# VIS4ROB-lab/ccm_slam

Hardware: AMD Instinct MI355X
Metric: global-BA LM iterations/s (4-agent merged map) (higher is better)
Workload: dtype f64; 1 GPU; gba_c4: global BA (MapFusionGBA numerics), 2000 KFs / 150000 landmarks / 954782 observations, Huber sqrt(5.99), landmark-sharded x1

## Files before the change

### ccm_slam_amd/csrc/ba_build.hip

```cpp
#include "common.h"
#include "ba_types.h"
#include "ba_math.h"
#include <algorithm>
#include <chrono>
#include <cstring>
#include <rocprim/rocprim.hpp>

int ccm_ba_build_pairs(ccm_ctx* ctx, const int* d_pt_off, const int* d_cslot, int Lp, int Cp, int lb, int le, int eb,
                       uint32_t** d_U_out, int* nOff_out, int** d_inst_off, int** d_inst_a, int** d_inst_c, int64_t* n_inst,
                       std::vector<std::pair<void*, size_t>>& keep);
int ccm_ba_pers_grid_fits(ccm_ctx* ctx, int grid);
int ccm_ba_state_from_raw(ccm_ba* ba);

namespace {

constexpr int kB = 256;

inline double now_ms() { return std::chrono::duration<double, std::milli>(std::chrono::steady_clock::now().time_since_epoch()).count(); }

struct BuildSizes {
  int Cp, Lp, Eact, bad, max_cam_edges, n_fix_edges, worst_units, n_units, pers_bad, n_ucol, n_cij, ncb, pad[4];
};

#define BB_RC(x) do { int rc_ = (x); if (rc_) return rc_; } while (0)
#define BB_HIP(x) do { hipError_t e_ = (x); if (e_ != hipSuccess) return ccm_set_error(ctx, CCM_E_HIP, std::string(#x) + ": " + hipGetErrorString(e_)); } while (0)

struct Tmp {
  ccm_ctx* ctx;
  std::vector<std::pair<void*, size_t>> blocks;
  template <typename T> int get(size_t n, T** out) {
    void* p = nullptr; size_t actual = 0;
    if (int rc = ccm_pool_get(ctx, std::max<size_t>(n, 1) * sizeof(T), &p, &actual)) return rc;
    blocks.push_back({p, actual});
    *out = (T*)p;
    return CCM_OK;
  }
  ~Tmp() { hipStreamSynchronize(ctx->stream); for (auto& b : blocks) ccm_pool_put(ctx, b.first, b.second); }
};

template <typename T>
int keep_get(ccm_ba* ba, size_t n, T** out, bool zero = false) {
  ccm_ctx* ctx = ba->ctx;
  void* p = nullptr; size_t actual = 0;
  const size_t bytes = std::max<size_t>(n, 1) * sizeof(T);
  if (int rc = ccm_pool_get(ctx, bytes, &p, &actual)) return rc;
  ba->allocs.push_back({p, actual});
  if (zero) ba->zero_list.push_back({p, bytes});
  *out = (T*)p;
  return CCM_OK;
}

constexpr int kZeroMax = 96;
constexpr unsigned kZeroChunk16 = 4096;
struct ZeroTab { void* p[kZeroMax]; unsigned n16[kZeroMax]; unsigned first_chunk[kZeroMax + 1]; int n; };
__global__ __launch_bounds__(256) void bb_zero_many(ZeroTab tab) {
  int k = 0;
  while (k + 1 < tab.n && blockIdx.x >= tab.first_chunk[k + 1]) k++;
  const unsigned c = blockIdx.x - tab.first_chunk[k];
  uint4* q = reinterpret_cast<uint4*>(tab.p[k]);
  const unsigned end = min(tab.n16[k], (c + 1) * kZeroChunk16);
  for (unsigned i = c * kZeroChunk16 + threadIdx.x; i < end; i += 256) q[i] = make_uint4(0u, 0u, 0u, 0u);
}
int flush_zero_list(ccm_ba* ba) {
  ccm_ctx* ctx = ba->ctx;
  size_t k = 0;
  while (k < ba->zero_list.size()) {
    ZeroTab tab;
    tab.n = 0;
    unsigned chunks = 0;
    for (; k < ba->zero_list.size() && tab.n < kZeroMax; k++) {
      const size_t n16 = (ba->zero_list[k].second + 15) / 16;
      if (n16 > 0xffffffffull / 2) { BB_HIP(hipMemsetAsync(ba->zero_list[k].first, 0, ba->zero_list[k].second, ctx->stream)); continue; }
      tab.p[tab.n] = ba->zero_list[k].first; tab.n16[tab.n] = (unsigned)n16; tab.first_chunk[tab.n] = chunks;
      chunks += (unsigned)((n16 + kZeroChunk16 - 1) / kZeroChunk16);
      tab.n++;
    }
    tab.first_chunk[tab.n] = chunks;
    if (chunks) hipLaunchKernelGGL(bb_zero_many, dim3(chunks), dim3(256), 0, ctx->stream, tab);
    BB_HIP(hipGetLastError());
  }
  ba->zero_list.clear();
  return CCM_OK;
}

int scan_excl(ccm_ctx* ctx, Tmp& tmp, const int* in, int* out, size_t n) {
  size_t bytes = 0;
  BB_HIP(rocprim::exclusive_scan(nullptr, bytes, in, out, 0, n, rocprim::plus<int>(), ctx->stream));
  char* scratch = nullptr;
  BB_RC(tmp.get(bytes, &scratch));
  BB_HIP(rocprim::exclusive_scan(scratch, bytes, in, out, 0, n, rocprim::plus<int>(), ctx->stream));
  return CCM_OK;
}

template <typename K>
int sort_pairs(ccm_ctx* ctx, Tmp& tmp, K* keys, int* vals, size_t n, unsigned bits, K** keys_sorted, int** vals_sorted) {
  *keys_sorted = keys; *vals_sorted = vals;
  if (n == 0) return CCM_OK;
  K* k2 = nullptr; int* v2 = nullptr;
  BB_RC(tmp.get(n, &k2)); BB_RC(tmp.get(n, &v2));
  rocprim::double_buffer<K> kb(keys, k2);
  rocprim::double_buffer<int> vb(vals, v2);
  size_t bytes = 0;
  BB_HIP(rocprim::radix_sort_pairs(nullptr, bytes, kb, vb, (unsigned)n, 0u, bits, ctx->stream));
  char* scratch = nullptr;
  BB_RC(tmp.get(bytes, &scratch));
  BB_HIP(rocprim::radix_sort_pairs(scratch, bytes, kb, vb, (unsigned)n, 0u, bits, ctx->stream));
  *keys_sorted = kb.current(); *vals_sorted = vb.current();
  return CCM_OK;
}

inline unsigned bits_for(uint64_t n_values) {
  unsigned b = 1;
  while (b < 63 && ((uint64_t)1 << b) < n_values) b++;
  return b;
}

__global__ void bb_mark(int n_edge, const int* ecam, const int* ept, const uint8_t* lvl, int n_cam, int n_pt, int* cam_has, int* pt_has, BuildSizes* sz) {
  const int e = blockIdx.x * blockDim.x + threadIdx.x;
  if (e >= n_edge) return;
  const int c = ecam[e], p = ept[e];
  if (c < 0 || c >= n_cam || p < 0 || p >= n_pt) { sz->bad = 1; return; }
  if (lvl && lvl[e] != 0) return;
  cam_has[c] = 1; pt_has[p] = 1;
}

__global__ void bb_flags(int n, const int* has, const uint8_t* fixed, int* flag) {
  const int i = blockIdx.x * blockDim.x + threadIdx.x;
  if (i > n) return;
  flag[i] = (i < n && has[i] && !(fixed && fixed[i])) ? 1 : 0;
}

__global__ void bb_slots(int n, const int* flag, const int* pre, int* slot, int* inv, int* total) {
  const int i = blockIdx.x * blockDim.x + threadIdx.x;
  if (i > n) return;
  if (i == n) { *total = pre[n]; return; }
  const int f = flag[i];
  slot[i] = f ? pre[i] : -1;
  if (f) inv[pre[i]] = i;
}

__global__ void bb_keys(int n_edge, const int* ecam, const int* ept, const uint8_t* lvl, int n_cam, int n_pt, const int* cam_slot, const int* pt_slot, unsigned cb,
                        unsigned pb, unsigned long long* keys, int* vals) {
  const int e = blockIdx.x * blockDim.x + threadIdx.x;
  if (e >= n_edge) return;
  const bool in_range = ecam[e] >= 0 && ecam[e] < n_cam && ept[e] >= 0 && ept[e] < n_pt;
  const bool act = in_range && !(lvl && lvl[e] != 0);
  unsigned long long k = (((unsigned long long)1 << (pb + cb)) - 1ull);
  if (act) k = ((unsigned long long)(unsigned)pt_slot[ept[e]] << cb) | (unsigned long long)(unsigned)(cam_slot[ecam[e]] + 1);
  keys[e] = k;
  vals[e] = e;
}

__global__ void bb_ptoff(int n_edge, const unsigned long long* keys, unsigned cb, unsigned pb, int* pt_off, int* cslot_g, BuildSizes* sz) {
  const int k = blockIdx.x * blockDim.x + threadIdx.x;
  if (k >= n_edge) return;
  const unsigned long long sent = ((unsigned long long)1 << pb) - 1ull;
  const unsigned long long cur = keys[k] >> cb;
  if (cur == sent) return;
  cslot_g[k] = (int)(keys[k] & (((unsigned long long)1 << cb) - 1ull)) - 1;
  const unsigned long long nxt = (k + 1 < n_edge) ? (keys[k + 1] >> cb) : sent;
  if (nxt != cur) pt_off[cur + 1] = k + 1;
  if (nxt == sent) sz->Eact = k + 1;
}

__global__ void bb_weights(int Lp, const int* pt_off, const int* cslot_g, long long* w) {
  const int l = blockIdx.x * blockDim.x + threadIdx.x;
  if (l >= Lp) return;
  int kf = 0;
  for (int k = pt_off[l]; k < pt_off[l + 1]; k++) kf += cslot_g[k] >= 0;
  w[l] = (long long)kf * (kf + 1) / 2 + (pt_off[l + 1] - pt_off[l]);
}

__global__ void bb_ptoff_local(int n, const int* g_pt_off, int eb, int* pt_off) {
  const int l = blockIdx.x * blockDim.x + threadIdx.x;
  if (l < n) pt_off[l] = g_pt_off[l] - eb;
}

__global__ void bb_gather(int Eloc, int eb, int lb, const unsigned long long* keys, const int* vals, unsigned cb, const int* ecam, const double* obs_raw,
                          const double* info_raw, int* ed_cam, int* ed_cslot, int* ed_pt, double* obs, double* info, int* loc_orig, unsigned* ckey, int* cval) {
  const int k = blockIdx.x * blockDim.x + threadIdx.x;
  if (k >= Eloc) return;
  const unsigned long long key = keys[eb + k];
  const int e = vals[eb + k];
  const int cs = (int)(key & (((unsigned long long)1 << cb) - 1ull)) - 1;
  ed_cam[k] = ecam[e]; ed_cslot[k] = cs; ed_pt[k] = (int)(key >> cb) - lb;
  obs[2 * (size_t)k] = obs_raw[2 * (size_t)e]; obs[2 * (size_t)k + 1] = obs_raw[2 * (size_t)e + 1];
  info[k] = info_raw[e];
  loc_orig[k] = e;
  ckey[k] = (unsigned)(cs + 1); cval[k] = k;
}

__global__ void bb_lower_bound(const unsigned* a, int n, int nq, int* off) {
  const int s = blockIdx.x * blockDim.x + threadIdx.x;
  if (s >= nq) return;
  int lo = 0, hi = n;
  while (lo < hi) { const int mid = (lo + hi) >> 1; if (a[mid] < (unsigned)s) lo = mid + 1; else hi = mid; }
  off[s] = lo;
}

__global__ void bb_cam_lists(int Eloc, const int* off_all , const int* cval, const int* ed_pt, int* cam_edge, int* cam_pt) {
  const int q = blockIdx.x * blockDim.x + threadIdx.x;
  const int nfix = off_all[1];
  if (q >= Eloc - nfix) return;
  const int k = cval[nfix + q];
  cam_edge[q] = k; cam_pt[q] = ed_pt[k];
}
__global__ void bb_cam_oi_bounded(int Eloc, const int* __restrict__ off_all, const int* __restrict__ cam_edge, const double* __restrict__ obs, const double* __restrict__ info,
                                  double* __restrict__ cam_oi) {
  const int s = blockIdx.x * blockDim.x + threadIdx.x;
  if (s >= Eloc - off_all[1]) return;
  const int e = cam_edge[s];
  typedef double v2d __attribute__((ext_vector_type(2)));
  v2d a, b; a[0] = obs[2 * (size_t)e]; a[1] = obs[2 * (size_t)e + 1]; b[0] = info[e]; b[1] = 0.0;
  reinterpret_cast<v2d*>(cam_oi)[2 * (size_t)s] = a; reinterpret_cast<v2d*>(cam_oi)[2 * (size_t)s + 1] = b;
}
__global__ void bb_cam_off(int Cp, const int* off_all, int* cam_off, BuildSizes* sz) {
  const int i = blockIdx.x * blockDim.x + threadIdx.x;
  if (i > Cp) return;
  cam_off[i] = off_all[i + 1] - off_all[1];
  if (i < Cp) atomicMax(&sz->max_cam_edges, off_all[i + 2] - off_all[i + 1]);
  if (i == 0) sz->n_fix_edges = off_all[1];
}

__global__ void bb_block_ij(int nOff, const uint32_t* U, int Cp, int* bi, int* bj, unsigned* jkey, int* jval) {
  const int b = blockIdx.x * blockDim.x + threadIdx.x;
  if (b >= nOff) return;
  const uint32_t u = U[b];
  const int i = (int)(u / (uint32_t)Cp), j = (int)(u % (uint32_t)Cp);
  bi[Cp + b] = i; bj[Cp + b] = j;
  jkey[b] = (unsigned)j; jval[b] = b;
}
__global__ void bb_diag_ij(int Cp, int* bi, int* bj) {
  const int i = blockIdx.x * blockDim.x + threadIdx.x;
  if (i < Cp) { bi[i] = i; bj[i] = i; }
}
__global__ void bb_rowblk_off(int Cp, const uint32_t* U, int nOff, int* rowblk_off) {
  const int i = blockIdx.x * blockDim.x + threadIdx.x;
  if (i > Cp) return;
  const unsigned long long key = (unsigned long long)i * (unsigned long long)Cp;
  int lo = 0, hi = nOff;
  while (lo < hi) { const int mid = (lo + hi) >> 1; if ((unsigned long long)U[mid] < key) lo = mid + 1; else hi = mid; }
  rowblk_off[i] = lo;
}
__global__ void bb_row_off(int Cp, const int* rowblk_off, const int* low_off, int* row_off) {
  const int i = blockIdx.x * blockDim.x + threadIdx.x;
  if (i <= Cp) row_off[i] = i + rowblk_off[i] + low_off[i];
}
__global__ void bb_row_fill(int Cp, int nOff, const int* bi, const int* bj, const unsigned* jkey_sorted, const int* jval_sorted, const int* rowblk_off,
                            const int* low_off, const int* row_off, int* row_col, uint32_t* row_blk) {
  const int t = blockIdx.x * blockDim.x + threadIdx.x;
  if (t < nOff) {
    {
      const int j = (int)jkey_sorted[t], b = jval_sorted[t];
      const int pos = row_off[j] + (t - low_off[j]);
      row_col[pos] = bi[Cp + b]; row_blk[pos] = (uint32_t)(Cp + b) | kTransposeBit;
    }
    {
      const int i = bi[Cp + t];
      const int pos = row_off[i] + (low_off[i + 1] - low_off[i]) + 1 + (t - rowblk_off[i]);
      row_col[pos] = bj[Cp + t]; row_blk[pos] = (uint32_t)(Cp + t);
    }
  }
  if (t < Cp) {
    const int pos = row_off[t] + (low_off[t + 1] - low_off[t]);
    row_col[pos] = t; row_blk[pos] = (uint32_t)t;
  }
}

__device__ __forceinline__ void pers_unit_rows(int u, int Cp, int& r0, int& r1) {
  r0 = min(Cp, (u >> 1) * kClu + (u & 1) * (kClu / 2));
  r1 = min(min(Cp, r0 + kClu / 2), ((u >> 1) + 1) * kClu);
}
template <int FILL>
__global__ __launch_bounds__(kB) void bb_pers_units(int Cp, int n_words, const int* row_off, const int* row_col, int* ucnt, const int* uoff, int* ucol, int* loc,
                                                  BuildSizes* sz) {
  extern __shared__ unsigned bm[];
  unsigned* wpre = bm + n_words;
  __shared__ int s_tot;
  const int u = blockIdx.x, t = threadIdx.x;
  int r0, r1;
  pers_unit_rows(u, Cp, r0, r1);
  for (int w = t; w < n_words; w += kB) bm[w] = 0u;
  __syncthreads();
  const int e0 = row_off[r0], e1 = row_off[r1];
  for (int s = e0 + t; s < e1; s += kB) { const int c = row_col[s]; atomicOr(&bm[c >> 5], 1u << (c & 31)); }
  __syncthreads();
  if (t == 0) {
    int acc = 0;
    for (int w = 0; w < n_words; w++) { wpre[w] = (unsigned)acc; acc += __popc(bm[w]); }
    s_tot = acc;
  }
  __syncthreads();
  if (!FILL) {
    if (t == 0) { ucnt[u] = s_tot; if (s_tot > kPersColCap || e1 - e0 > kPersIdxCap) sz->pers_bad = 1; }
    return;
  }
  const int base = uoff[u];
  for (int w = t; w < n_words; w += kB) {
    unsigned m = bm[w];
    int pos = base + (int)wpre[w];
    while (m) { const int b = __ffs(m) - 1; ucol[pos++] = 32 * w + b; m &= m - 1; }
  }
  for (int s = e0 + t; s < e1; s += kB) { const int c = row_col[s]; loc[s] = (int)wpre[c >> 5] + __popc(bm[c >> 5] & ((1u << (c & 31)) - 1u)); }
}

template <int FILL>
__global__ __launch_bounds__(kB) void bb_cluster_entries(int Cp, const int* row_off, const int* row_col, const uint32_t* row_blk, int* ccnt, const int* coff, int* cij,
                                                       uint32_t* cblk) {
  __shared__ int s_scan[kB];
  __shared__ int s_run;
  const int c = blockIdx.x, t = threadIdx.x;
  const int r0 = c * kClu, r1 = min(Cp, r0 + kClu);
  const int e0 = row_off[r0], e1 = row_off[r1];
  if (t == 0) s_run = 0;
  __syncthreads();
  for (int sb = e0; sb < e1; sb += kB) {
    const int s = sb + t;
    int col = -1;
    if (s < e1) col = row_col[s];
    const int in = (s < e1 && col >= r0 && col < r1) ? 1 : 0;
    s_scan[t] = in;
    __syncthreads();
    for (int off = 1; off < kB; off <<= 1) {
      const int v = (t >= off) ? s_scan[t - off] : 0;
      __syncthreads();
      s_scan[t] += v;
      __syncthreads();
    }
    const int run = s_run;
    if (FILL && in) {
      int lo = r0, hi = r1;
      while (hi - lo > 1) { const int mid = (lo + hi) >> 1; if (row_off[mid] <= s) lo = mid; else hi = mid; }
      const int pos = coff[c] + run + s_scan[t] - 1;
      cij[pos] = ((lo - r0) << 4) | (col - r0);
      cblk[pos] = row_blk[s];
    }
    __syncthreads();
    if (t == kB - 1) s_run = run + s_scan[kB - 1];
    __syncthreads();
  }
  if (!FILL && t == 0) ccnt[c] = s_run;
}

__global__ void bb_unit_counts(int nOff, int chunk, const int* inst_off, int* nub) {
  const int t = blockIdx.x * blockDim.x + threadIdx.x;
  if (t <= nOff) nub[t] = (t < nOff) ? max(1, (inst_off[t + 1] - inst_off[t] + chunk - 1) / chunk) : 0;
}
__global__ void bb_unit_offsets(int nOff, int Cp, const int* blk_pref, const int* rowblk_off, int* row_unit_off, int* blk_unit0, BuildSizes* sz) {
  const int t = blockIdx.x * blockDim.x + threadIdx.x;
  if (t <= Cp) row_unit_off[t] = blk_pref[rowblk_off[t]];
  if (t < Cp) atomicMax(&sz->worst_units, blk_pref[rowblk_off[t + 1]] - blk_pref[rowblk_off[t]]);
  if (t == 0) sz->n_units = blk_pref[nOff];
  if (t <= nOff) blk_unit0[t] = blk_pref[t];
}
__global__ __launch_bounds__(kB) void bb_unit_fill(int Cp, int chunk, const int* rowblk_off, const int* inst_off, const int* row_unit_off, const int* blk_unit0, int4* tab) {
  extern __shared__ int su[];
  const int i = blockIdx.x, t = threadIdx.x;
  const int base = row_unit_off[i], n = row_unit_off[i + 1] - base;
  int* blk = su; int* s0a = su + n; int* s1a = su + 2 * n;
  for (int b = rowblk_off[i] + t; b < rowblk_off[i + 1]; b += kB) {
    int c = blk_unit0[b] - base, s0 = inst_off[b];
    const int end = inst_off[b + 1];
    do { const int s1 = min(end, s0 + chunk); blk[c] = b; s0a[c] = s0; s1a[c] = s1; c++; s0 = s1; } while (s0 < end);
  }
  __syncthreads();
  for (int c = t; c < n; c += kB) {
    const int len = s1a[c] - s0a[c];
    int rank = 0;
    for (int o = 0; o < n; o++) { const int lo = s1a[o] - s0a[o]; rank += (lo > len || (lo == len && o < c)) ? 1 : 0; }
    tab[base + rank] = make_int4(blk[c], s0a[c], s1a[c], c);
  }
}

__global__ void bb_edge_rank(const int* cam_off, const int* cam_edge, int* rank) {
  const int i = blockIdx.x;
  for (int s = cam_off[i] + threadIdx.x; s < cam_off[i + 1]; s += blockDim.x) rank[cam_edge[s]] = s - cam_off[i];
}
__global__ void bb_inst_rank(const int* inst_a, const int* rank, int n, int* inst_al) {
  const int s = blockIdx.x * blockDim.x + threadIdx.x;
  if (s < n) inst_al[s] = rank[inst_a[s]];
}
__global__ void bb_edge_cpos(const int* cam_off, const int* cam_edge, int* cpos) {
  const int i = blockIdx.x;
  for (int s = cam_off[i] + threadIdx.x; s < cam_off[i + 1]; s += blockDim.x) cpos[cam_edge[s]] = s;
}
__global__ void bb_inst_cpos(const int* inst_c, const int* cpos, int n, int* inst_cp) {
  const int s = blockIdx.x * blockDim.x + threadIdx.x;
  if (s < n) inst_cp[s] = cpos[inst_c[s]];
}

__global__ void bb_coarse_keys(int Cp, int nOff, const int* bi, const int* bj, int na, int agg, unsigned* keys, int* vals) {
  const int k = blockIdx.x * blockDim.x + threadIdx.x;
  if (k >= Cp + nOff) return;
  const int a = bi[k] / agg, a2 = bj[k] / agg;
  keys[k] = (unsigned)a * (unsigned)na + (unsigned)a2;
  vals[k] = (k < Cp) ? 2 * k : 2 * k + (a == a2 ? 1 : 0);
}
__global__ void bb_coarse_ab(const unsigned* uniq, const int* n_runs, int na, int* cb_ab, BuildSizes* sz) {
  const int r = blockIdx.x * blockDim.x + threadIdx.x;
  if (r == 0) sz->ncb = *n_runs;
  if (r >= *n_runs) return;
  cb_ab[2 * r] = (int)(uniq[r] / (unsigned)na); cb_ab[2 * r + 1] = (int)(uniq[r] % (unsigned)na);
}
__global__ void bb_counts_tail(unsigned* counts, const int* n_runs) { counts[*n_runs] = 0u; }

__global__ void bb_state_init(int n_cam, int Lloc, int lb, const double* raw_cam, const double* raw_pt, const int* slot_pt, double* cam0, double* cam1, double* pt0,
                              double* pt1) {
  const int t = blockIdx.x * blockDim.x + threadIdx.x;
  if (t < n_cam) {
// ... 422 lines not shown
```

### ccm_slam_amd/csrc/ba_structure.hip

```cpp
#include "common.h"
#include <cstring>
#include <rocprim/rocprim.hpp>
#include <vector>

namespace {

constexpr int kTPB = 256;

template <int EMIT>
__global__ void pairs_kernel(const int* pt_off, const int* cslot, int l0, int n_l, int Cp, int* cnt, const int* poff, uint32_t* keys,
                             unsigned long long* vals) {
  const int i = blockIdx.x * blockDim.x + threadIdx.x;
  if (i >= n_l) return;
  const int l = l0 + i;
  const int k0 = pt_off[l], k1 = pt_off[l + 1];
  int n = 0;
  int w = EMIT ? poff[i] : 0;
  for (int a = k0; a < k1; a++) {
    const int ia = cslot[a];
    if (ia < 0) continue;
    for (int c = a + 1; c < k1; c++) {
      const int ic = cslot[c];
      if (ic == ia) continue;
      if (EMIT) { keys[w] = (uint32_t)ia * (uint32_t)Cp + (uint32_t)ic; if (vals) vals[w] = ((unsigned long long)(uint32_t)a << 32) | (uint32_t)c; w++; }
      n++;
    }
  }
  if (!EMIT) cnt[i] = n;
}

__global__ void split_kernel(const unsigned long long* vals, int n, int eb, int* inst_a, int* inst_c) {
  const int i = blockIdx.x * blockDim.x + threadIdx.x;
  if (i >= n) return;
  inst_a[i] = (int)(vals[i] >> 32) - eb;
  inst_c[i] = (int)(uint32_t)vals[i] - eb;
}

__global__ void ranges_kernel(const uint32_t* U, int nOff, const uint32_t* own_keys, int n_own, int* inst_off) {
  const int b = blockIdx.x * blockDim.x + threadIdx.x;
  if (b > nOff) return;
  if (b == nOff) { inst_off[b] = n_own; return; }
  const uint32_t key = U[b];
  int lo = 0, hi = n_own;
  while (lo < hi) { const int mid = (lo + hi) >> 1; if (own_keys[mid] < key) lo = mid + 1; else hi = mid; }
  inst_off[b] = lo;
}

struct Tmp {
  ccm_ctx* ctx;
  std::vector<std::pair<void*, size_t>> blocks;
  template <typename T> int get(size_t n, T** out) {
    void* p = nullptr; size_t actual = 0;
    if (int rc = ccm_pool_get(ctx, std::max<size_t>(n, 1) * sizeof(T), &p, &actual)) return rc;
    blocks.push_back({p, actual});
    *out = (T*)p;
    return CCM_OK;
  }
  ~Tmp() { hipStreamSynchronize(ctx->stream); for (auto& b : blocks) ccm_pool_put(ctx, b.first, b.second); }
};

#define ST_RC(x) do { int rc_ = (x); if (rc_) return rc_; } while (0)
#define ST_HIP(x) do { hipError_t e_ = (x); if (e_ != hipSuccess) return ccm_set_error(ctx, CCM_E_HIP, std::string(#x) + ": " + hipGetErrorString(e_)); } while (0)

int emit_pairs(ccm_ctx* ctx, Tmp& tmp, const int* d_pt_off, const int* d_cslot, int l0, int l1, int Cp, bool with_vals, uint32_t** keys,
               unsigned long long** vals, int* n_out) {
  const int n_l = l1 - l0;
  *keys = nullptr; if (vals) *vals = nullptr; *n_out = 0;
  if (n_l <= 0) return CCM_OK;
  int *cnt = nullptr, *poff = nullptr;
  ST_RC(tmp.get((size_t)n_l + 1, &cnt)); ST_RC(tmp.get((size_t)n_l + 1, &poff));
  ST_HIP(hipMemsetAsync(cnt + n_l, 0, sizeof(int), ctx->stream));
  hipLaunchKernelGGL(pairs_kernel<0>, dim3(ccm_div_up(n_l, kTPB)), dim3(kTPB), 0, ctx->stream, d_pt_off, d_cslot, l0, n_l, Cp, cnt, (const int*)nullptr,
                     (uint32_t*)nullptr, (unsigned long long*)nullptr);
  size_t bytes = 0;
  ST_HIP(rocprim::exclusive_scan(nullptr, bytes, cnt, poff, 0, (size_t)n_l + 1, rocprim::plus<int>(), ctx->stream));
  char* scratch = nullptr;
  ST_RC(tmp.get(bytes, &scratch));
  ST_HIP(rocprim::exclusive_scan(scratch, bytes, cnt, poff, 0, (size_t)n_l + 1, rocprim::plus<int>(), ctx->stream));
  int total = 0;
  ST_HIP(hipMemcpyAsync(&total, poff + n_l, sizeof(int), hipMemcpyDeviceToHost, ctx->stream));
  ST_HIP(hipStreamSynchronize(ctx->stream));
  *n_out = total;
  if (total == 0) return CCM_OK;
  ST_RC(tmp.get((size_t)total, keys));
  if (with_vals) ST_RC(tmp.get((size_t)total, vals));
  hipLaunchKernelGGL(pairs_kernel<1>, dim3(ccm_div_up(n_l, kTPB)), dim3(kTPB), 0, ctx->stream, d_pt_off, d_cslot, l0, n_l, Cp, (int*)nullptr, (const int*)poff,
                     *keys, with_vals ? *vals : (unsigned long long*)nullptr);
  ST_HIP(hipGetLastError());
  return CCM_OK;
}

}

int ccm_ba_build_pairs(ccm_ctx* ctx, const int* d_pt_off, const int* d_cslot, int Lp, int Cp, int lb, int le, int eb,
                       uint32_t** d_U_out, int* nOff_out, int** d_inst_off, int** d_inst_a, int** d_inst_c, int64_t* n_inst,
                       std::vector<std::pair<void*, size_t>>& keep) {
  if (Cp > 65535) return ccm_set_error(ctx, CCM_E_ARG, "bundle adjustment: more than 65535 free cameras (32-bit block keys)");
  *n_inst = 0; *nOff_out = 0; *d_U_out = nullptr;
  auto keep_get = [&](size_t n, int** out) -> int {
    void* p = nullptr; size_t actual = 0;
    if (int rc = ccm_pool_get(ctx, std::max<size_t>(n, 1) * sizeof(int), &p, &actual)) return rc;
    keep.push_back({p, actual}); *out = (int*)p; return CCM_OK;
  };
  Tmp tmp{ctx, {}};
  unsigned bits = 1;
  while (bits < 32 && ((uint64_t)1 << bits) < (uint64_t)Cp * (uint64_t)Cp) bits++;
  const bool whole = (lb == 0 && le == Lp);
  uint32_t* ok = nullptr; unsigned long long* ov = nullptr; int n_own = 0;
  ST_RC(emit_pairs(ctx, tmp, d_pt_off, d_cslot, lb, le, Cp, true, &ok, &ov, &n_own));
  uint32_t* ok_sorted = ok; unsigned long long* ov_sorted = ov;
  if (n_own) {
    uint32_t* ok2 = nullptr; unsigned long long* ov2 = nullptr;
    ST_RC(tmp.get((size_t)n_own, &ok2)); ST_RC(tmp.get((size_t)n_own, &ov2));
    rocprim::double_buffer<uint32_t> kb(ok, ok2);
    rocprim::double_buffer<unsigned long long> vb(ov, ov2);
    size_t bytes = 0;
    ST_HIP(rocprim::radix_sort_pairs(nullptr, bytes, kb, vb, (unsigned)n_own, 0u, bits, ctx->stream));
    char* scratch = nullptr;
    ST_RC(tmp.get(bytes, &scratch));
    ST_HIP(rocprim::radix_sort_pairs(scratch, bytes, kb, vb, (unsigned)n_own, 0u, bits, ctx->stream));
    ok_sorted = kb.current(); ov_sorted = vb.current();
  }
  uint32_t* gk_sorted = ok_sorted; int n_all = n_own;
  if (!whole) {
    uint32_t* gk = nullptr;
    ST_RC(emit_pairs(ctx, tmp, d_pt_off, d_cslot, 0, Lp, Cp, false, &gk, nullptr, &n_all));
    gk_sorted = gk;
    if (n_all) {
      uint32_t* gk2 = nullptr;
      ST_RC(tmp.get((size_t)n_all, &gk2));
      rocprim::double_buffer<uint32_t> kb(gk, gk2);
      size_t bytes = 0;
      ST_HIP(rocprim::radix_sort_keys(nullptr, bytes, kb, (unsigned)n_all, 0u, bits, ctx->stream));
      char* scratch = nullptr;
      ST_RC(tmp.get(bytes, &scratch));
      ST_HIP(rocprim::radix_sort_keys(scratch, bytes, kb, (unsigned)n_all, 0u, bits, ctx->stream));
      gk_sorted = kb.current();
    }
  }
  int nOff = 0;
  uint32_t* U = nullptr; unsigned* counts = nullptr; int* runs = nullptr;
  if (n_all) {
    ST_RC(tmp.get((size_t)n_all, &U)); ST_RC(tmp.get((size_t)n_all, &counts)); ST_RC(tmp.get(1, &runs));
    size_t bytes = 0;
    ST_HIP(rocprim::run_length_encode(nullptr, bytes, gk_sorted, (unsigned)n_all, U, counts, runs, ctx->stream));
    char* scratch = nullptr;
    ST_RC(tmp.get(bytes, &scratch));
    ST_HIP(rocprim::run_length_encode(scratch, bytes, gk_sorted, (unsigned)n_all, U, counts, runs, ctx->stream));
    ST_HIP(hipMemcpyAsync(&nOff, runs, sizeof(int), hipMemcpyDeviceToHost, ctx->stream));
    ST_HIP(hipStreamSynchronize(ctx->stream));
  }
  int* U_keep = nullptr;
  ST_RC(keep_get((size_t)nOff, &U_keep));
  if (nOff) ST_HIP(hipMemcpyAsync(U_keep, U, (size_t)nOff * sizeof(uint32_t), hipMemcpyDeviceToDevice, ctx->stream));
  ST_RC(keep_get((size_t)nOff + 1, d_inst_off)); ST_RC(keep_get((size_t)n_own, d_inst_a)); ST_RC(keep_get((size_t)n_own, d_inst_c));
  hipLaunchKernelGGL(ranges_kernel, dim3(ccm_div_up(nOff + 1, kTPB)), dim3(kTPB), 0, ctx->stream, (const uint32_t*)U, nOff, (const uint32_t*)ok_sorted, n_own,
                     *d_inst_off);
  if (n_own) hipLaunchKernelGGL(split_kernel, dim3(ccm_div_up(n_own, kTPB)), dim3(kTPB), 0, ctx->stream, (const unsigned long long*)ov_sorted, n_own, eb, *d_inst_a, *d_inst_c);
  ST_HIP(hipGetLastError());
  *d_U_out = (uint32_t*)U_keep;
  *nOff_out = nOff;
  *n_inst = n_own;
  return CCM_OK;
}
```

Measured before the change: 971.8 LM iter/s.

## Parallelise pair emission across observations and force onesweep radix sort for large arrays

The one-thread-per-landmark pair emit kernel is replaced with a block-tiled kernel. Each tile of observations computes per-row pair counts, does a shared-memory prefix scan and hands pairs out to threads by binary search, which balances work across landmarks with long tracks. The count kernel now uses a closed-form count instead of the nested loop. Radix sorts above 2^18 elements select a rocprim config that disables the merge-sort fallback so onesweep is used, with an env override. These are build-time structure steps, so any effect on per-iteration LM throughput depends on whether the build is inside the timed region.

```diff
diff --git a/ccm_slam_amd/csrc/ba_build.hip b/ccm_slam_amd/csrc/ba_build.hip
--- a/ccm_slam_amd/csrc/ba_build.hip
+++ b/ccm_slam_amd/csrc/ba_build.hip
@@ -1,6 +1,7 @@
 #include "common.h"
 #include "ba_types.h"
 #include "ba_math.h"
+#include "ba_sort.h"
 #include <algorithm>
 #include <chrono>
 #include <cstring>
@@ -100,11 +101,12 @@
   BB_RC(tmp.get(n, &k2)); BB_RC(tmp.get(n, &v2));
   rocprim::double_buffer<K> kb(keys, k2);
   rocprim::double_buffer<int> vb(vals, v2);
+  const bool onesweep = ba_sort_onesweep(n);
   size_t bytes = 0;
-  BB_HIP(rocprim::radix_sort_pairs(nullptr, bytes, kb, vb, (unsigned)n, 0u, bits, ctx->stream));
+  BB_HIP(ba_radix_sort_pairs(onesweep, nullptr, bytes, kb, vb, (unsigned)n, bits, ctx->stream));
   char* scratch = nullptr;
   BB_RC(tmp.get(bytes, &scratch));
-  BB_HIP(rocprim::radix_sort_pairs(scratch, bytes, kb, vb, (unsigned)n, 0u, bits, ctx->stream));
+  BB_HIP(ba_radix_sort_pairs(onesweep, scratch, bytes, kb, vb, (unsigned)n, bits, ctx->stream));
   *keys_sorted = kb.current(); *vals_sorted = vb.current();
   return CCM_OK;
 }
diff --git a/ccm_slam_amd/csrc/ba_sort.h b/ccm_slam_amd/csrc/ba_sort.h
--- /dev/null
+++ b/ccm_slam_amd/csrc/ba_sort.h
@@ -0,0 +1,26 @@
+#pragma once
+#include <cstdlib>
+#include <cstring>
+#include <rocprim/rocprim.hpp>
+
+constexpr size_t kBaOnesweepFrom = ((size_t)1 << 18) + 1;
+
+using BaSortNoMerge = rocprim::radix_sort_config<rocprim::default_config, rocprim::default_config, rocprim::default_config, 0>;
+
+inline bool ba_sort_onesweep(size_t n) {
+  const char* s = getenv("CCM_BA_SORT");
+  if (s && !strcmp(s, "merge")) return false;
+  if (s && !strcmp(s, "onesweep")) return true;
+  return n >= kBaOnesweepFrom;
+}
+
+template <typename K, typename V>
+inline hipError_t ba_radix_sort_pairs(bool onesweep, void* scratch, size_t& bytes, rocprim::double_buffer<K>& kb, rocprim::double_buffer<V>& vb, unsigned n, unsigned bits,
+                                      hipStream_t st) {
+  return onesweep ? rocprim::radix_sort_pairs<BaSortNoMerge>(scratch, bytes, kb, vb, n, 0u, bits, st)
+                  : rocprim::radix_sort_pairs(scratch, bytes, kb, vb, n, 0u, bits, st);
+}
+template <typename K>
+inline hipError_t ba_radix_sort_keys(bool onesweep, void* scratch, size_t& bytes, rocprim::double_buffer<K>& kb, unsigned n, unsigned bits, hipStream_t st) {
+  return onesweep ? rocprim::radix_sort_keys<BaSortNoMerge>(scratch, bytes, kb, n, 0u, bits, st) : rocprim::radix_sort_keys(scratch, bytes, kb, n, 0u, bits, st);
+}
diff --git a/ccm_slam_amd/csrc/ba_structure.hip b/ccm_slam_amd/csrc/ba_structure.hip
--- a/ccm_slam_amd/csrc/ba_structure.hip
+++ b/ccm_slam_amd/csrc/ba_structure.hip
@@ -1,4 +1,5 @@
 #include "common.h"
+#include "ba_sort.h"
 #include <cstring>
 #include <rocprim/rocprim.hpp>
 #include <vector>
@@ -7,26 +8,74 @@
 
 constexpr int kTPB = 256;
 
-template <int EMIT>
-__global__ void pairs_kernel(const int* pt_off, const int* cslot, int l0, int n_l, int Cp, int* cnt, const int* poff, uint32_t* keys,
-                             unsigned long long* vals) {
+__device__ __forceinline__ int row_same(const int* __restrict__ cslot, int a, int k1, int ia) {
+  int d = 0;
+  while (a + 1 + d < k1 && cslot[a + 1 + d] == ia) d++;
+  return d;
+}
+
+__global__ void pairs_count_kernel(const int* __restrict__ pt_off, const int* __restrict__ cslot, int l0, int n_l, int* __restrict__ cnt) {
   const int i = blockIdx.x * blockDim.x + threadIdx.x;
   if (i >= n_l) return;
-  const int l = l0 + i;
-  const int k0 = pt_off[l], k1 = pt_off[l + 1];
+  const int k1 = pt_off[l0 + i + 1];
   int n = 0;
-  int w = EMIT ? poff[i] : 0;
-  for (int a = k0; a < k1; a++) {
+  for (int a = pt_off[l0 + i]; a < k1; a++) {
     const int ia = cslot[a];
-    if (ia < 0) continue;
-    for (int c = a + 1; c < k1; c++) {
-      const int ic = cslot[c];
-      if (ic == ia) continue;
-      if (EMIT) { keys[w] = (uint32_t)ia * (uint32_t)Cp + (uint32_t)ic; if (vals) vals[w] = ((unsigned long long)(uint32_t)a << 32) | (uint32_t)c; w++; }
-      n++;
-    }
-  }
-  if (!EMIT) cnt[i] = n;
+    if (ia >= 0) n += k1 - 1 - a - row_same(cslot, a, k1, ia);
+  }
+  cnt[i] = n;
+}
+
+constexpr int kEmitLm = 32;
+__global__ __launch_bounds__(kTPB) void pairs_emit_kernel(const int* __restrict__ pt_off, const int* __restrict__ cslot, int l0, int n_l, int Cp,
+                                                          const int* __restrict__ poff, uint32_t* __restrict__ keys, unsigned long long* __restrict__ vals) {
+  __shared__ int s_off[kEmitLm + 1];
+  __shared__ int s_cs[kTPB];
+  __shared__ int s_skip[kTPB];
+  __shared__ int s_row[kTPB + 1];
+  const int t = threadIdx.x;
+  const int i0 = blockIdx.x * kEmitLm, nl = min(kEmitLm, n_l - i0);
+  for (int j = t; j <= nl; j += kTPB) s_off[j] = pt_off[l0 + i0 + j];
+  __syncthreads();
+  const int e0 = s_off[0], e1 = s_off[nl];
+  int w = poff[i0];
+  for (int r0 = e0; r0 < e1; r0 += kTPB) {
+    const int nr = min(kTPB, e1 - r0);
+    if (t < nr) s_cs[t] = cslot[r0 + t];
+    __syncthreads();
+    auto cs = [&](int x) { return x - r0 < nr ? s_cs[x - r0] : cslot[x]; };
+    int len = 0, d = 0;
+    if (t < nr) {
+      const int a = r0 + t, ia = s_cs[t];
+      if (ia >= 0) {
+        int lo = 0, hi = nl;
+        while (hi - lo > 1) { const int mid = (lo + hi) >> 1; if (s_off[mid] <= a) lo = mid; else hi = mid; }
+        const int k1 = s_off[lo + 1];
+        while (a + 1 + d < k1 && cs(a + 1 + d) == ia) d++;
+        len = k1 - 1 - a - d;
+      }
+      s_skip[t] = d;
+    }
+    s_row[t + 1] = len;
+    if (t == 0) s_row[0] = 0;
+    __syncthreads();
+    for (int off = 1; off < kTPB; off <<= 1) {
+      const int v = (t >= off) ? s_row[t + 1 - off] : 0;
+      __syncthreads();
+      s_row[t + 1] += v;
+      __syncthreads();
+    }
+    const int n_tile = s_row[kTPB];
+    for (int p = t; p < n_tile; p += kTPB) {
+      int lo = 0, hi = nr;
+      while (hi - lo > 1) { const int mid = (lo + hi) >> 1; if (s_row[mid] <= p) lo = mid; else hi = mid; }
+      const int a = r0 + lo, c = a + 1 + s_skip[lo] + (p - s_row[lo]);
+      keys[w + p] = (uint32_t)s_cs[lo] * (uint32_t)Cp + (uint32_t)cs(c);
+      if (vals) vals[w + p] = ((unsigned long long)(uint32_t)a << 32) | (uint32_t)c;
+    }
+    w += n_tile;
+    __syncthreads();
+  }
 }
 
 __global__ void split_kernel(const unsigned long long* vals, int n, int eb, int* inst_a, int* inst_c) {
@@ -70,8 +119,7 @@
   int *cnt = nullptr, *poff = nullptr;
   ST_RC(tmp.get((size_t)n_l + 1, &cnt)); ST_RC(tmp.get((size_t)n_l + 1, &poff));
   ST_HIP(hipMemsetAsync(cnt + n_l, 0, sizeof(int), ctx->stream));
-  hipLaunchKernelGGL(pairs_kernel<0>, dim3(ccm_div_up(n_l, kTPB)), dim3(kTPB), 0, ctx->stream, d_pt_off, d_cslot, l0, n_l, Cp, cnt, (const int*)nullptr,
-                     (uint32_t*)nullptr, (unsigned long long*)nullptr);
+  hipLaunchKernelGGL(pairs_count_kernel, dim3(ccm_div_up(n_l, kTPB)), dim3(kTPB), 0, ctx->stream, d_pt_off, d_cslot, l0, n_l, cnt);
   size_t bytes = 0;
   ST_HIP(rocprim::exclusive_scan(nullptr, bytes, cnt, poff, 0, (size_t)n_l + 1, rocprim::plus<int>(), ctx->stream));
   char* scratch = nullptr;
@@ -84,8 +132,8 @@
   if (total == 0) return CCM_OK;
   ST_RC(tmp.get((size_t)total, keys));
   if (with_vals) ST_RC(tmp.get((size_t)total, vals));
-  hipLaunchKernelGGL(pairs_kernel<1>, dim3(ccm_div_up(n_l, kTPB)), dim3(kTPB), 0, ctx->stream, d_pt_off, d_cslot, l0, n_l, Cp, (int*)nullptr, (const int*)poff,
-                     *keys, with_vals ? *vals : (unsigned long long*)nullptr);
+  hipLaunchKernelGGL(pairs_emit_kernel, dim3((unsigned)ccm_div_up(n_l, kEmitLm)), dim3(kTPB), 0, ctx->stream, d_pt_off, d_cslot, l0, n_l, Cp,
+                     (const int*)poff, *keys, with_vals ? *vals : (unsigned long long*)nullptr);
   ST_HIP(hipGetLastError());
   return CCM_OK;
 }
@@ -114,11 +162,12 @@
     ST_RC(tmp.get((size_t)n_own, &ok2)); ST_RC(tmp.get((size_t)n_own, &ov2));
     rocprim::double_buffer<uint32_t> kb(ok, ok2);
     rocprim::double_buffer<unsigned long long> vb(ov, ov2);
+    const bool onesweep = ba_sort_onesweep((size_t)n_own);
     size_t bytes = 0;
-    ST_HIP(rocprim::radix_sort_pairs(nullptr, bytes, kb, vb, (unsigned)n_own, 0u, bits, ctx->stream));
+    ST_HIP(ba_radix_sort_pairs(onesweep, nullptr, bytes, kb, vb, (unsigned)n_own, bits, ctx->stream));
     char* scratch = nullptr;
     ST_RC(tmp.get(bytes, &scratch));
-    ST_HIP(rocprim::radix_sort_pairs(scratch, bytes, kb, vb, (unsigned)n_own, 0u, bits, ctx->stream));
+    ST_HIP(ba_radix_sort_pairs(onesweep, scratch, bytes, kb, vb, (unsigned)n_own, bits, ctx->stream));
     ok_sorted = kb.current(); ov_sorted = vb.current();
   }
   uint32_t* gk_sorted = ok_sorted; int n_all = n_own;
@@ -130,11 +179,12 @@
       uint32_t* gk2 = nullptr;
       ST_RC(tmp.get((size_t)n_all, &gk2));
       rocprim::double_buffer<uint32_t> kb(gk, gk2);
+      const bool onesweep = ba_sort_onesweep((size_t)n_all);
       size_t bytes = 0;
-      ST_HIP(rocprim::radix_sort_keys(nullptr, bytes, kb, (unsigned)n_all, 0u, bits, ctx->stream));
+      ST_HIP(ba_radix_sort_keys(onesweep, nullptr, bytes, kb, (unsigned)n_all, bits, ctx->stream));
       char* scratch = nullptr;
       ST_RC(tmp.get(bytes, &scratch));
-      ST_HIP(rocprim::radix_sort_keys(scratch, bytes, kb, (unsigned)n_all, 0u, bits, ctx->stream));
+      ST_HIP(ba_radix_sort_keys(onesweep, scratch, bytes, kb, (unsigned)n_all, bits, ctx->stream));
       gk_sorted = kb.current();
     }
   }
```

Result: faster. 986.9 LM iter/s (median of 6 runs) (+1.6%).
